# seungju-k1m/Distributed_RL

Measured on AMD Instinct MI355X. Metric: learner frames/sec (whole node), Ape-X DQN Atari CNN, higher is better.
Workload: dtype bf16; 1 GPU; model=ape_x net (ape_x.json), global_batch=512, seq_len=4, parallelism=dp1, actors=0, replay=gpu sum-tree PER, graph=True

## Files before the change

distributed_rl_amd/algos/ape_x.py:

```python

from __future__ import annotations

import os as _os
import time
from collections import deque
from typing import Any, Dict, List, Optional

import numpy as np
import torch

from .. import ops
from ..config import Config
from ..models import BaseAgent
from ..models.base_agent import CNN2D
from ..replay import make_apex_schema, make_per
from .common import LearnerBase

PUBLISH_EVERY = 50
ACTOR_PULL_EVERY = 100


class ApexLearner(LearnerBase):
    ALG = "APE_X"

# ... 408 lines not shown
            t_hid = self._t_pre_hidden_of if pre else self._t_hidden_of
            h_s = hid(f_s)
            with torch.no_grad():
                h_on = hid(f_on)
                h_tg = t_hid(f_tg)
            wa, ba, wv, bv = self._head_params
            wat, bat, wvt, bvt = self._thead_params
            loss, prio, qmean = ops.dueling_q_head_loss(
                h_s, wa, ba, wv, bv, h_on, h_tg, wat, bat, wvt, bvt,
                actions, rewards, dones, weights, self.gamma, self.n_step,
                self.alpha, pre_act=pre,
            )
        elif cuda and getattr(self, "_fast_heads", None) is not None:
            adv_s, val_s = self._fast_heads(s)
            with torch.no_grad():
                adv_on, val_on = self._fast_heads(sp)
                adv_tg, val_tg = self._target_heads(sp)
            loss, prio, qmean = ops.dueling_nstep_dqn_loss(
                adv_s, val_s, adv_on, val_on, adv_tg, val_tg, actions,
                rewards, dones, weights, self.gamma, self.n_step, self.alpha,
            )
        else:
            q_s = self._online_q(s) if cuda else self.net.forward([s])[0]
            with torch.no_grad():
                q_sp_on = (self._online_q(sp) if cuda
                           else self.net.forward([sp])[0])
                q_sp_tg = self.target.forward([sp])[0]
            loss, prio, qmean = ops.nstep_dqn_loss(
                q_s, q_sp_on, q_sp_tg, actions, rewards,
                dones, weights, self.gamma, self.n_step, self.alpha,
                with_value_stat=True,
            )
        if self.mp is not None:
            self.mp.direct_grads(loss, getattr(self, "_direct_list", None))
        else:
            self.optim.zero_grad(set_to_none=False)
            loss.backward()
        return {"loss": loss.detach(), "value": qmean}, prio

    def _optimize_mp(self):
        if (_os.environ.get("DRL_FUSED_OPT_TAIL", "1") == "1"
                and self.mp.fused_step(self.optim)):
            return
        self.mp.upcast_grads()
        self.optim.step()
        self.mp.sync_compute_params()

    def sync_target(self):
        if self.mp is not None:
            self.flat_tparam.copy_(self.mp.flat_cparam)
        else:
            self.target.updateParameter(self.model, 1.0)

    def _inner_step(self) -> Dict[str, torch.Tensor]:
        data, idx, w = self.replay.sample(self.batch_size, self.beta)
        return self.train_step(data, idx, w)

    def _cadence(self):
        self.step_count += 1
        if self.step_count % self.cfg.target_frequency == 0:
            self.sync_target()
            self.publish_weights(include_target=True)
        elif self.step_count % PUBLISH_EVERY == 0:
            self.publish_weights()

    def step(self) -> Dict[str, torch.Tensor]:
        stats = self.maybe_profile_first_step(self._inner_step)
# ... 425 lines not shown
```

distributed_rl_amd/ops/__init__.py:

```python

from __future__ import annotations

import os
from typing import Optional

import torch

from . import torch_ref

_EXT = None
_EXT_TRIED = False


def hip_ext(required: bool = True):
    global _EXT, _EXT_TRIED
    if _EXT is None and not _EXT_TRIED:
        _EXT_TRIED = True
        from . import build as _build

        _EXT = _build.load_prebuilt()
        if _EXT is None and torch.cuda.is_available():
            try:
                _EXT = _build.build()
            except Exception as e:
                if required:
                    raise RuntimeError(
                        "gfx950 HIP extension missing and build failed: %s" % e
                    )
    if _EXT is None and required and not _allow_eager():
        raise RuntimeError(
            "device tensor reached a fused op but the _drl_hip extension is "
            "not built; run `python -m distributed_rl_amd.ops.build` "
            "(or set DRL_ALLOW_EAGER=1 to debug with eager torch)"
        )
    return _EXT
# ... 10 lines not shown
    return ext is not None




def dequant_frames(x_u8: torch.Tensor, dtype: torch.dtype = torch.bfloat16) -> torch.Tensor:
    if _use_hip(x_u8):
        out = torch.empty(x_u8.shape, dtype=dtype, device=x_u8.device)
        hip_ext().dequant(x_u8.contiguous(), out)
        return out
    return torch_ref.dequant_frames(x_u8, dtype)


def dequant_frames_nhwc(x_u8: torch.Tensor) -> torch.Tensor:
    if _use_hip(x_u8):
        out = torch.empty(
            x_u8.shape, dtype=torch.bfloat16, device=x_u8.device,
            memory_format=torch.channels_last,
        )
        hip_ext().dequant_nhwc(x_u8.contiguous(), out)
        return out
    return torch_ref.dequant_frames(x_u8, torch.float32).to(
        memory_format=torch.channels_last
    )




def conv_supported(H, W, C, KH, KW, S, COUT, u8: bool, chw_out: bool = False,
                   njobs: int = 1) -> bool:
    ext = hip_ext(required=False)
    return ext is not None and bool(
        ext.conv_fwd_supported(H, W, C, KH, KW, S, COUT, u8, chw_out, njobs))


def _fused_conv_backward(x, weight, out, gout, stride, has_bias, chw, pq,
                         need_x, need_w, need_b):
    COUT = weight.shape[0]
    if chw:
        P, Q = pq
        N = gout.shape[0]
        masked = torch.empty(N, COUT, P, Q, dtype=torch.bfloat16,
                             device=gout.device,
                             memory_format=torch.channels_last)
        hip_ext().relu_mask_bwd_chw(gout.contiguous(), out, masked,
                                    COUT, P * Q)
        gout = masked
    else:
        if not gout.is_contiguous(memory_format=torch.channels_last):
            gout = gout.contiguous(memory_format=torch.channels_last)
        masked = torch.empty_like(gout)
        hip_ext().relu_mask_bwd(gout, out, masked)
        gout = masked
    COUT, C, KH, KW = weight.shape
    ext = hip_ext()
    use_own_wrw = need_w and bool(
        ext.conv_wrw_supported(x.shape[2], x.shape[3], C, KH, KW, stride,
                               COUT, x.dtype == torch.uint8)
    )
    gw = gb = None
    if use_own_wrw and os.environ.get("DRL_WRW_BF16", "1") == "1":
        gw = torch.empty(COUT, KH, KW, C, dtype=torch.bfloat16,
                         device=x.device).permute(0, 3, 1, 2)
        gb = (torch.empty(COUT, dtype=torch.bfloat16, device=x.device)
              if need_b else None)
        ext.conv_wrw(x, gout, gw,
                     gb if need_b else torch.empty(0, device=x.device),
                     stride)
    elif use_own_wrw:
        K = KH * KW * C
        flat_ws = torch.empty(COUT * (K + 1), dtype=torch.float32,
                              device=x.device)
        ws = flat_ws[: COUT * K].view(COUT, K)
        gb_ws = (flat_ws[COUT * K :] if need_b
                 else torch.empty(0, device=x.device))
        ext.conv_wrw(x, gout, ws, gb_ws, stride)
        gw = ws.view(COUT, KH, KW, C).permute(0, 3, 1, 2).to(torch.bfloat16)
        if need_b:
            gb = gb_ws.to(torch.bfloat16)
    gi = None
    use_own_dgrad = (
        os.environ.get("DRL_OWN_DGRAD", "0") == "1"
        and need_x and x.dtype == torch.bfloat16
        and bool(ext.conv_dgrad_supported(x.shape[2], x.shape[3], C, KH,
                                          KW, stride, COUT))
    )
    if use_own_dgrad:
        gi = torch.empty_like(x)
        w_t = torch.empty(weight.numel(), dtype=torch.bfloat16,
                          device=x.device)
        ext.conv_dgrad(gout, weight, w_t, gi, stride)
    if (need_x and not use_own_dgrad) or (need_w and not use_own_wrw):
        if x.dtype == torch.uint8:
            xf = dequant_frames(x.permute(0, 2, 3, 1), torch.bfloat16)
            xf = xf.permute(0, 3, 1, 2)
        else:
            xf = x
        gi2, gw2, gb2 = torch.ops.aten.convolution_backward(
            gout, xf, weight,
            [COUT] if has_bias else None,
            [stride, stride], [0, 0], [1, 1], False, [0, 0], 1,
# ... 63 lines not shown
                continue
            x, weight, out = saved[k : k + 3]
            k += 3
            if gouts[j] is None:
                continue
            need_x = ctx.needs_input_grad[3 + j]
            need_w = ctx.needs_input_grad[3 + n + j]
            need_b = ctx.has_bias and ctx.needs_input_grad[3 + 2 * n + j]
            gi, gw, gb = _fused_conv_backward(
                x, weight, out, gouts[j], ctx.stride, ctx.has_bias, ctx.chw,
                ctx.pq, need_x, need_w, need_b)
            grads[j], grads[n + j], grads[2 * n + j] = gi, gw, gb
        return (None, None, None, *grads)


def fused_conv_relu_grouped(xs, weights, biases, stride: int,
                            chw_out: bool = False):
    n = len(xs)
    assert len(weights) == n and len(biases) == n
    return _FusedConvGroupedFn.apply(stride, bool(chw_out), n, *xs, *weights,
                                     *biases)


def fused_conv_relu(x, weight, bias, stride: int, chw_out: bool = False):
    return _FusedConvGroupedFn.apply(stride, bool(chw_out), 1, x, weight,
                                     bias)[0]




def conv3x3_supported(H, W, C, COUT) -> bool:
    ext = hip_ext(required=False)
    return ext is not None and bool(ext.conv3x3p1_supported(H, W, C, COUT))


def _gate(name: str, default: bool) -> bool:
    v = os.environ.get(name)
    if v is None or v == "":
        return default
    return v == "1"


_RESCONV_WRW_DEFAULT = True
_RESCONV_DGRAD_DEFAULT = True


class _FusedConv3x3Fn(torch.autograd.Function):

    @staticmethod
    def forward(ctx, x, weight, bias, residual, relu_in, relu_out):
        ext = hip_ext()
        N, _, H, W = x.shape
        COUT = weight.shape[0]
        empty = torch.empty(0, device=x.device, dtype=torch.bfloat16)
        out = torch.empty(
            N, COUT, H, W, dtype=torch.bfloat16, device=x.device,
            memory_format=torch.channels_last,
        )
        ext.conv3x3p1_fwd(x, weight, bias if bias is not None else empty,
                          residual if residual is not None else empty, out,
                          relu_in, relu_out)
        ctx.save_for_backward(x, weight, out if relu_out else None)
        ctx.has_bias = bias is not None
        ctx.relu_in = relu_in
        ctx.relu_out = relu_out
        return out

    @staticmethod
    def backward(ctx, gout):
        x, weight, out = ctx.saved_tensors
        ext = hip_ext()
        COUT = weight.shape[0]
        if not gout.is_contiguous(memory_format=torch.channels_last):
# ... 676 lines not shown
```

distributed_rl_amd/ops/hip/conv_mfma.hip:

```cpp

#include <hip/hip_runtime.h>
#include <atomic>
#include <hip/hip_bf16.h>
#include <torch/extension.h>
#include <ATen/cuda/CUDAContext.h>

namespace {

using bf16x8 = __attribute__((ext_vector_type(8))) __bf16;
using f32x4 = __attribute__((ext_vector_type(4))) float;

constexpr int kPad = 32;

template <int H, int W, int C, int KH, int KW, int S, int COUT, bool U8IN>
struct ConvGeom {
  static constexpr int P = (H - KH) / S + 1;
  static constexpr int Q = (W - KW) / S + 1;
  static constexpr int K = KH * KW * C;
  static constexpr int KCHUNKS = K / 32;
  static_assert(K % 32 == 0, "K must be a multiple of 32");
  static_assert((KW * C) % 32 == 0, "patch row must tile by 32");
  static constexpr int ROWC = KW * C;
  static constexpr int LDS_ROW = K + kPad;
  static constexpr int LDS_ELEMS = COUT * LDS_ROW;
};

template <int H, int W, int C, int KH, int KW, int S, int COUT, bool U8IN,
          int WAVES, int RPW, bool CHW_OUT = false>
__device__ __forceinline__ void conv_fwd_block(
    const void* __restrict__ in_v,
    const __bf16* __restrict__ weight,
    const __bf16* __restrict__ bias,
    __bf16* __restrict__ out,
    int batch, int tile, __bf16* wlds) {
  using G = ConvGeom<H, W, C, KH, KW, S, COUT, U8IN>;
// ... 250 lines not shown
        bf16x8 v;
        if (m < M) {
          v = *reinterpret_cast<const bf16x8*>(gout + (int64_t)m * COUT + c0);
        } else {
#pragma unroll
          for (int j = 0; j < 8; ++j) v[j] = (__bf16)0.0f;
        }
        *reinterpret_cast<bf16x8*>(g_t + (piece / PIECES) * GSTRIDE + c0) = v;
      }
    }
    __syncthreads();
    bf16x8 bfrag = tr_frag<ASTRIDE>(a_t, lane, wave);
#pragma unroll
    for (int cb = 0; cb < CBLK; ++cb) {
      bf16x8 afrag = tr_frag<GSTRIDE>(g_t, lane, cb);
      acc[cb] = __builtin_amdgcn_mfma_f32_16x16x32_bf16(afrag, bfrag, acc[cb],
                                                        0, 0, 0);
    }
    __syncthreads();
  }

  float* plane = gw_part + (int64_t)mb * (COUT * G::K + kPlanePad);
  const int kout = ktile * 64 + wave * 16 + (lane & 15);
#pragma unroll
  for (int cb = 0; cb < CBLK; ++cb)
#pragma unroll
    for (int r = 0; r < 4; ++r) {
      const int cout = cb * 16 + (lane >> 4) * 4 + r;
      plane[(int64_t)cout * G::K + kout] = acc[cb][r];
    }
}

template <typename OutT>
__global__ __launch_bounds__(256) void wrw_reduce_kernel(
    const float* __restrict__ part, int planes, int n_elem,
    OutT* __restrict__ out, const float* __restrict__ b_part, int b_planes,
    int cout, OutT* __restrict__ b_out) {
  __shared__ __attribute__((aligned(16))) float sh4_raw[256 * 4];
  float* sh = sh4_raw;
  const int tid = threadIdx.x;
  const int e_blocks = (n_elem + 63) / 64;
  if ((int)blockIdx.x < e_blocks) {
    const int e4 = blockIdx.x * 64 + (tid & 15) * 4;
    const int g = tid >> 4;
    float4 s = {0.0f, 0.0f, 0.0f, 0.0f};
    const float4 zero = {0.0f, 0.0f, 0.0f, 0.0f};
    for (int p = g; p < planes; p += 64) {
      float4 v[4];
#pragma unroll
      for (int u = 0; u < 4; ++u) {
        const int pu = p + 16 * u;
        v[u] = pu < planes ? *reinterpret_cast<const float4*>(
                                 part + (int64_t)pu * (n_elem + kPlanePad) + e4)
                           : zero;
      }
#pragma unroll
      for (int u = 0; u < 4; ++u) {
        s.x += v[u].x; s.y += v[u].y; s.z += v[u].z; s.w += v[u].w;
      }
    }
    float4* sh4 = reinterpret_cast<float4*>(sh4_raw);
    sh4[tid] = s;
    __syncthreads();
    if (tid < 16) {
      float4 t = sh4[tid];
      for (int k = 1; k < 16; ++k) {
        const float4 v = sh4[k * 16 + tid];
        t.x += v.x; t.y += v.y; t.z += v.z; t.w += v.w;
      }
      if constexpr (std::is_same<OutT, float>::value) {
        *reinterpret_cast<float4*>(out + e4) = t;
      } else {
        v4bf_w o = {(__bf16)t.x, (__bf16)t.y, (__bf16)t.z, (__bf16)t.w};
        *reinterpret_cast<v4bf_w*>(out + e4) = o;
      }
    }
  } else {
    const int G = 256 / cout;
    const int c = tid % cout, g = tid / cout;
    float s = 0.0f;
    for (int p = g; p < b_planes; p += G) s += b_part[p * cout + c];
    sh[tid] = s;
    __syncthreads();
    if (tid < cout) {
      float t = 0.0f;
      for (int k = 0; k < G; ++k) t += sh[k * cout + tid];
      b_out[tid] = (OutT)t;
    }
  }
}

template <int COUT>
__global__ __launch_bounds__(256) void colsum_bf16_kernel(
    const __bf16* __restrict__ x, int64_t M, float* __restrict__ out) {
  typedef __bf16 bf8 __attribute__((ext_vector_type(8)));
  __shared__ float sh[256 * 8];
  const int tid = threadIdx.x;
  const int64_t nchunk = M * COUT / 8;
  int64_t i = (int64_t)blockIdx.x * blockDim.x + tid;
  const int64_t stride = (int64_t)gridDim.x * blockDim.x;
  float acc[8] = {0, 0, 0, 0, 0, 0, 0, 0};
  const bf8* __restrict__ x8 = (const bf8*)x;
  for (; i < nchunk; i += stride) {
    bf8 v = x8[i];
#pragma unroll
    for (int j = 0; j < 8; ++j) acc[j] += (float)v[j];
  }
#pragma unroll
  for (int j = 0; j < 8; ++j) sh[tid * 8 + j] = acc[j];
  __syncthreads();
  if (tid < COUT) {
    float s = 0.0f;
    for (int t = tid >> 3; t < 256; t += COUT / 8) s += sh[t * 8 + (tid & 7)];
    out[(int64_t)blockIdx.x * COUT + tid] = s;
  }
}

}

namespace {
typedef __bf16 v4bf __attribute__((ext_vector_type(4)));
__global__ void tr16_probe_kernel(float* out, int mode) {
  __shared__ __bf16 lds[512];
  int lane = threadIdx.x & 63;
  for (int i = threadIdx.x; i < 512; i += 64) lds[i] = (__bf16)(float)i;
  __syncthreads();
  int off;
  switch (mode) {
    case 0: off = 0; break;
    case 1: off = lane * 4; break;
    case 2: off = (lane >> 4) * 64; break;
    default: off = (lane & 15) * 4; break;
  }
  auto* p = (__attribute__((address_space(3))) v4bf*)(lds + off);
  v4bf v = __builtin_amdgcn_ds_read_tr16_b64_v4bf16(p);
#pragma unroll
  for (int j = 0; j < 4; ++j) out[lane * 4 + j] = (float)v[j];
}
}

namespace {

template <int H, int W, int C, int KH, int KW, int S, int COUT, int WAVES,
          int RPW>
__global__ __launch_bounds__(WAVES * 64) void conv_dgrad_kernel(
    const __bf16* __restrict__ gout,
    const __bf16* __restrict__ w_t,
    __bf16* __restrict__ dx,
    int batch) {
// ... 1205 lines not shown
}

constexpr int kMaxDevices = 64;

int resident_blocks(std::atomic<int>* per_dev, const void* fn, int lds_bytes,
                    const char* who) {
  const int dev = at::cuda::current_device();
  TORCH_CHECK(dev >= 0 && dev < kMaxDevices, who, ": device index");
  std::atomic<int>& slot = per_dev[dev];
  int r = slot.load(std::memory_order_relaxed);
  if (r == 0) {
    int per_cu = 0;
    TORCH_CHECK(hipOccupancyMaxActiveBlocksPerMultiprocessor(
                    &per_cu, fn, 256, lds_bytes) == hipSuccess && per_cu > 0,
                who, ": occupancy query failed");
    r = per_cu * at::cuda::getCurrentDeviceProperties()->multiProcessorCount;
    slot.store(r, std::memory_order_relaxed);
  }
  return r;
}

int wrw_resident_blocks(const Conv3Launch& L) {
  static std::atomic<int> cache[std::size(kConv3Launches)][kMaxDevices] = {};
  return resident_blocks(cache[&L - kConv3Launches], (const void*)L.wrw,
                         L.wrw_lds_bytes, "conv3x3p1_wrw");
}

int wrw_resident_blocks(const StemLaunch& L) {
  static std::atomic<int> cache[std::size(kStemLaunches)][kMaxDevices] = {};
  return resident_blocks(cache[&L - kStemLaunches], (const void*)L.wrw,
                         L.wrw_lds_bytes, "conv3x3c4_wrw");
}

void launch_wrw_fold(const torch::Tensor& part, int mb,
                     const torch::Tensor& gout, int M, int64_t COUT,
                     void (*colsum)(const __bf16*, int64_t, float*),
                     torch::Tensor& gw_ws, torch::Tensor& gb_ws, bool bias) {
  constexpr int kColsumBlocks = 256;
  auto st = cur_stream();
  const int n_elem = (int)gw_ws.numel();
  const bool bf16_out = gw_ws.scalar_type() == kBF16;
  torch::Tensor b_part;
  if (bias) {
    b_part = torch::empty({(int64_t)kColsumBlocks, COUT}, part.options());
    hipLaunchKernelGGL(colsum, dim3(kColsumBlocks), dim3(256), 0, st,
                       (const __bf16*)gout.data_ptr(), (int64_t)M,
                       b_part.data_ptr<float>());
  }
  const int e_blocks = (n_elem + 63) / 64;
  const float* b_part_ptr =
      bias ? (const float*)b_part.data_ptr<float>() : nullptr;
  if (bf16_out)
    hipLaunchKernelGGL(wrw_reduce_kernel<__bf16>,
                       dim3(e_blocks + (bias ? 1 : 0)), dim3(256), 0, st,
                       (const float*)part.data_ptr<float>(), mb, n_elem,
                       (__bf16*)gw_ws.data_ptr(), b_part_ptr, kColsumBlocks,
                       (int)COUT, bias ? (__bf16*)gb_ws.data_ptr() : nullptr);
  else
    hipLaunchKernelGGL(wrw_reduce_kernel<float>,
                       dim3(e_blocks + (bias ? 1 : 0)), dim3(256), 0, st,
                       (const float*)part.data_ptr<float>(), mb, n_elem,
                       gw_ws.data_ptr<float>(), b_part_ptr, kColsumBlocks,
                       (int)COUT, bias ? gb_ws.data_ptr<float>() : nullptr);
}

struct Conv3Labels {
  const char *in, *out, *bias, *residual, *mask;
};

void launch_conv3(const torch::Tensor& in, const __bf16* w,
                  const __bf16* flip_from, const torch::Tensor& bias,
                  const torch::Tensor& residual, const torch::Tensor& mask,
                  const torch::Tensor& out, int64_t COUT, bool relu_in,
                  bool relu_out, const Conv3Labels& lb) {
  const int64_t N = in.size(0), C = in.size(1), H = in.size(2), W = in.size(3);
  check_nhwc(in, kBF16, N, C, H, W, lb.in);
  check_nhwc(out, kBF16, N, COUT, H, W, lb.out);
  TORCH_CHECK(out.data_ptr() != in.data_ptr(), lb.out, " must not alias ",
              lb.in, " (not in-place)");
  TORCH_CHECK((uintptr_t)in.data_ptr() % 16 == 0, lb.in, " is misaligned");
  TORCH_CHECK((uintptr_t)w % 16 == 0, lb.in, "'s weight is misaligned");
// ... 57 lines not shown
                      std::vector<torch::Tensor> biases,
                      std::vector<torch::Tensor> outs, int64_t stride,
                      bool chw_out) {
  const size_t njobs = ins.size();
  TORCH_CHECK(njobs >= 1 && njobs <= kMaxConvJobs, "1..", kMaxConvJobs,
              " conv jobs per launch");
  TORCH_CHECK(weights.size() == njobs && outs.size() == njobs &&
                  (biases.empty() || biases.size() == njobs),
              "conv_fwd_grouped wants one weight, output and bias per job");
  const Geom g = geom_of(ins[0], weights[0], stride);
  const ConvEntry* e = find_geom(kConvs, g);
  TORCH_CHECK(e, "no fused conv kernel for this geometry: ", g.H, "x", g.W,
              "x", g.C, " k", g.KH, "x", g.KW, " s", g.S, " -> ", g.COUT,
              " u8=", g.u8);
  launch_conv_fwd(*e, ins, weights, biases, outs, chw_out);
}

bool conv_fwd_variant(torch::Tensor in, torch::Tensor weight,
                      torch::Tensor bias, torch::Tensor out, int64_t stride,
                      int64_t variant) {
  if (variant < 0 || variant >= (int64_t)std::size(kVariants)) return false;
  const ConvEntry& e = kVariants[variant];
  if (!(e.g == geom_of(in, weight, stride))) return false;
  launch_conv_fwd(e, {in}, {weight}, {bias}, {out}, false);
  return true;
}

bool conv_wrw_supported(int64_t H, int64_t W, int64_t C, int64_t KH, int64_t KW,
                        int64_t S, int64_t COUT, bool u8) {
  const ConvEntry* e = find_conv(H, W, C, KH, KW, S, COUT, u8);
  return e && e->wrw;
}

void conv_wrw(torch::Tensor in, torch::Tensor gout, torch::Tensor gw_ws,
              torch::Tensor gb_ws, int64_t stride) {
  TORCH_CHECK(in.dim() == 4 && gout.dim() == 4 && stride >= 1,
              "conv_wrw wants 4-D in and gout and a positive stride");
  const int64_t N = in.size(0), C = in.size(1), H = in.size(2), W = in.size(3);
  const int64_t COUT = gout.size(1), P = gout.size(2), Q = gout.size(3);
  const bool u8 = in.scalar_type() == torch::kUInt8;
  const ConvEntry* L =
      find_conv(H, W, C, H - (P - 1) * stride, W - (Q - 1) * stride, stride,
                COUT, u8);
  TORCH_CHECK(L && L->wrw, "no wrw kernel for this geometry");
  check_nhwc(in, u8 ? torch::kUInt8 : kBF16, N, C, H, W, "conv_wrw in");
  check_nhwc(gout, kBF16, N, COUT, P, Q, "conv_wrw gout (in's batch)");
  const bool bf16_out = gw_ws.scalar_type() == kBF16;
  check_dev(gw_ws, bf16_out ? kBF16 : torch::kFloat32, "conv_wrw gw_ws");
  TORCH_CHECK(gw_ws.is_contiguous() ||
              (gw_ws.dim() == 4 &&
               gw_ws.is_contiguous(at::MemoryFormat::ChannelsLast)));
  const int n_elem = (int)gw_ws.numel();
  TORCH_CHECK(gw_ws.numel() == COUT * L->g.K(), "gw_ws shape mismatch");
  const bool bias = gb_ws.defined() && gb_ws.numel() > 0;
  if (bias) check_rows(gb_ws, gw_ws.scalar_type(), {COUT}, "conv_wrw gb_ws");
  const int M = checked_rows(N * P * Q, "conv_wrw");
  const int n_chunks = (M + 31) / 32;
  int mb = (n_chunks > 8192 ? 2048 : 512) / L->ktiles;
  if (mb > n_chunks) mb = n_chunks;
  if (mb < 1) mb = 1;
  auto st = cur_stream();
  const auto f32 = gw_ws.options().dtype(torch::kFloat32);
  auto part = torch::empty({(int64_t)mb, (int64_t)n_elem + kPlanePad}, f32);
  hipLaunchKernelGGL(L->wrw, dim3(L->ktiles, mb), dim3(256), L->wrw_lds_bytes,
                     st, (const void*)in.data_ptr(),
                     (const __bf16*)gout.data_ptr(), part.data_ptr<float>(),
                     (int)N, mb);
  launch_wrw_fold(part, mb, gout, M, COUT, L->colsum, gw_ws, gb_ws, bias);
}

bool conv_dgrad_supported(int64_t H, int64_t W, int64_t C, int64_t KH,
                          int64_t KW, int64_t S, int64_t COUT) {
  return find_geom(kDgrad, Geom{H, W, C, KH, KW, S, COUT, false}) != nullptr;
}

void conv_dgrad(torch::Tensor gout, torch::Tensor weight, torch::Tensor w_t,
                torch::Tensor dx, int64_t stride) {
  TORCH_CHECK(dx.dim() == 4 && weight.dim() == 4 && stride >= 1,
              "conv_dgrad wants 4-D dx and weight and a positive stride");
  const int64_t N = dx.size(0), C = dx.size(1), H = dx.size(2), W = dx.size(3);
  const int64_t COUT = weight.size(0), KH = weight.size(2), KW = weight.size(3);
  const DgradEntry* L =
      find_geom(kDgrad, Geom{H, W, C, KH, KW, stride, COUT, false});
  TORCH_CHECK(L, "no dgrad kernel for this geometry");
  check_nhwc(dx, kBF16, N, C, H, W, "conv_dgrad dx");
  check_nhwc(weight, kBF16, COUT, C, KH, KW, "conv_dgrad weight");
  check_nhwc(gout, kBF16, N, COUT, L->g.P(), L->g.Q(), "conv_dgrad gout");
  check_rows(w_t, kBF16, {weight.numel()}, "conv_dgrad w_t");
  const int M = checked_rows(N * H * W, "conv_dgrad");
  if (M == 0) return;
  auto stream = cur_stream();
  const int total = (int)weight.numel();
  hipLaunchKernelGGL(conv_w_transpose_kernel, dim3((total + 255) / 256),
                     dim3(256), 0, stream, (const __bf16*)weight.data_ptr(),
                     (__bf16*)w_t.data_ptr(), (int)(KH * KW), (int)C,
                     (int)COUT);
  const int rows_per_block = L->waves * L->rpw;
  const int blocks = (M + rows_per_block - 1) / rows_per_block;
  hipLaunchKernelGGL(L->fn, dim3(blocks), dim3(L->waves * 64), 0, stream,
                     (const __bf16*)gout.data_ptr(),
                     (const __bf16*)w_t.data_ptr(), (__bf16*)dx.data_ptr(),
                     (int)N);
// ... 268 lines not shown
  const int64_t N = gx.size(0), C = gx.size(1), H = gx.size(2), W = gx.size(3);
  TORCH_CHECK(maxpool3x3s2_supported(H, W, C),
              "no 3x3 s2 max-pool kernel for this geometry: ", H, "x", W, "x",
              C);
  const int64_t P = (H - 1) / 2 + 1, Q = (W - 1) / 2 + 1;
  check_nhwc(gout, kBF16, N, C, P, Q, "maxpool3x3s2_bwd gout");
  check_nhwc(idx, torch::kUInt8, N, C, P, Q, "maxpool3x3s2_bwd idx");
  check_nhwc(gx, kBF16, N, C, H, W, "maxpool3x3s2_bwd gx");
  TORCH_CHECK((uintptr_t)gout.data_ptr() % 16 == 0 &&
                  (uintptr_t)idx.data_ptr() % 16 == 0 &&
                  (uintptr_t)gx.data_ptr() % 16 == 0,
              "maxpool3x3s2_bwd: misaligned tensor");
  const int lanes = checked_rows(N * H * W * (C / 16), "maxpool3x3s2_bwd");
  if (lanes == 0) return;
  const dim3 grid((unsigned)(((int64_t)lanes + 255) / 256));
  hipLaunchKernelGGL(maxpool3x3s2_bwd_kernel, grid, dim3(256), 0, cur_stream(),
                     (const __bf16*)gout.data_ptr(),
                     (const uint8_t*)idx.data_ptr(), (__bf16*)gx.data_ptr(),
                     lanes, (int)H, (int)W, (int)P, (int)Q, (int)(C / 16));
}

void register_conv(pybind11::module_& m) {
  m.def("mfma_probe", &mfma_probe, "16x16x32 bf16 MFMA fragment-map probe");
  m.def("tr16_probe", &tr16_probe);
  m.def("conv_fwd_grouped", &conv_fwd_grouped,
        "fused NHWC bf16 MFMA conv fwd (+dequant on u8 input, bias, ReLU, "
        "optional flatten-fused CHW out) for 1..4 same-geometry jobs in one "
        "launch");
  m.def("conv_fwd_supported", &conv_fwd_supported);
  m.def("conv_fwd_variant", &conv_fwd_variant, "tuning-variant conv fwd");
  m.def("conv_wrw", &conv_wrw,
        "MFMA conv weight-grad; gw/gb are fp32 workspaces or bf16 grads");
  m.def("conv_wrw_supported", &conv_wrw_supported);
  m.def("conv_dgrad", &conv_dgrad,
        "MFMA conv data-grad (masked-tap gather, pre-transposed weights)");
  m.def("conv_dgrad_supported", &conv_dgrad_supported);
  m.def("relu_mask_bwd_chw", &relu_mask_bwd_chw,
        "relu-mask + CHW->NHWC transpose (backward of the fused flatten)");
  m.def("linear_relu", &linear_relu,
        "fused Linear+bias+ReLU fwd (own MFMA GEMM, LDS-staged W)");
  m.def("linear_relu_supported", &linear_relu_supported);
  m.def("conv3x3p1_fwd", &conv3x3p1_fwd,
        "MFMA 3x3 s1 pad-1 NHWC bf16 conv fwd (+relu_in, bias, residual, "
        "relu_out)");
  m.def("conv3x3p1_supported", &conv3x3p1_supported);
  m.def("conv3x3p1_wrw", &conv3x3p1_wrw,
        "MFMA 3x3 s1 pad-1 weight-grad (+relu_in); gw/gb are fp32 workspaces "
        "or bf16 grads");
  m.def("conv3x3p1_wrw_supported", &conv3x3p1_wrw_supported);
  m.def("conv3x3p1_dgrad", &conv3x3p1_dgrad,
        "3x3 s1 pad-1 input-grad: weight flip + the forward kernel at the "
        "mirrored geometry (+relu_in mask in the epilogue)");
  m.def("conv3x3c4_fwd", &conv3x3c4_fwd,
        "MFMA 3x3 s1 pad-1 NHWC bf16 stem conv fwd (84x84, C=4 -> 16; bias)");
  m.def("conv3x3c4_supported", &conv3x3c4_supported);
  m.def("conv3x3c4_wrw", &conv3x3c4_wrw,
        "MFMA stem-conv weight-grad, ordered planes; gw/gb are fp32 "
        "workspaces or bf16 grads");
  m.def("conv3x3c4_wrw_supported", &conv3x3c4_wrw_supported);
  m.def("maxpool3x3s2_fwd", &maxpool3x3s2_fwd,
        "NHWC bf16 max-pool 3x3 s2 pad-1 fwd; uint8 tap plane, or none when "
        "idx is empty");
  m.def("maxpool3x3s2_bwd", &maxpool3x3s2_bwd,
        "max-pool 3x3 s2 pad-1 input-grad: ordered gather over the tap "
        "plane, every gx element written once");
  m.def("maxpool3x3s2_supported", &maxpool3x3s2_supported);
// ... 2 lines not shown
```

distributed_rl_amd/ops/torch_ref.py:

```python

from __future__ import annotations

from typing import Tuple

import torch



def dequant_frames(x_u8: torch.Tensor, dtype: torch.dtype = torch.float32) -> torch.Tensor:
    return x_u8.to(dtype) / 255.0




def conv3x3_res(x, weight, bias=None, relu_in: bool = False,
                relu_out: bool = False, residual=None) -> torch.Tensor:
    y = torch.nn.functional.conv2d(
        torch.nn.functional.relu(x) if relu_in else x, weight, bias, padding=1)
    if residual is not None:
        y = y + residual
    return torch.nn.functional.relu(y) if relu_out else y



# ... 292 lines not shown
def sumtree_bump_seed(seed: int) -> int:
    return ((int(seed) & _U64) * 6364136223846793005
            + 1442695040888963407) & _U64


def sumtree_sample(tree, P: int, n_valid: int, k: int, seed: int):
    import numpy as np

    tree = np.asarray(tree, dtype=np.float32)
    assert tree.size == 2 * P and 1 <= n_valid <= P and k >= 1
    i = np.arange(k, dtype=np.int64)
    total = tree[1]
    u = (i.astype(np.float32) + sumtree_hash01(seed, i)) * (total / np.float32(k))
    node = np.ones(k, dtype=np.int64)
    level = 1
    while level < P:
        left_child = node << 1
        lv = tree[left_child]
        left = u < lv
        u = np.where(left, u, u - lv)
        node = np.where(left, left_child, left_child + 1)
        level <<= 1
    idx = np.minimum(node - P, n_valid - 1)
    prob = tree[P + idx] / total
    return idx, prob




def fold_nstep_reward(rewards: torch.Tensor, gamma: float) -> torch.Tensor:
    n = rewards.shape[-1]
    disc = gamma ** torch.arange(n, dtype=rewards.dtype, device=rewards.device)
    return (rewards * disc).sum(-1)
```

distributed_rl_amd/parallel/precision.py:

```python

from __future__ import annotations

import copy
from typing import Callable, Optional

import torch
import torch.distributed as dist


def _is_cl(p: torch.Tensor) -> bool:
    return p.dim() == 4 and p.is_contiguous(memory_format=torch.channels_last) \
        and not p.is_contiguous()


def _to_flat(p: torch.Tensor) -> torch.Tensor:
    if _is_cl(p):
        return p.permute(0, 2, 3, 1).reshape(-1)
    return p.reshape(-1)


def _view_like(flat_slice: torch.Tensor, p: torch.Tensor) -> torch.Tensor:
    if _is_cl(p):
        N, C, H, W = p.shape
        return flat_slice.view(N, H, W, C).permute(0, 3, 1, 2)
    return flat_slice.view_as(p)


class _Group:

    def __init__(self, dtype, c_params, m_params, device):
        self.dtype = dtype
        self.c_params = c_params
        self.m_params = m_params
        total = sum(p.numel() for p in c_params)
        self.flat_cparam = torch.empty(total, dtype=dtype, device=device)
# ... 66 lines not shown
                    f"params {names} are not adjacent in the flat buffer"
                )
                buf = g.flat_cparam if of == "param" else g.flat_cgrad
                return buf[start:end]
        raise KeyError(f"params {names} not found in one group")

    @property
    def flat_cparam(self):
        assert len(self.groups) == 1
        return self.groups[0].flat_cparam

    @property
    def flat_cgrad(self):
        assert len(self.groups) == 1
        return self.groups[0].flat_cgrad

    @property
    def flat_mgrad(self):
        assert len(self.groups) == 1
        return self.groups[0].flat_mgrad

    @property
    def flat_mparam(self):
        assert len(self.groups) == 1
        return self.groups[0].flat_mparam

    def all_mgrads(self):
        return [g.flat_mgrad for g in self.groups]

    def zero_grads(self):
        for g in self.groups:
            g.flat_cgrad.zero_()

    def direct_grads(self, loss, params_override=None):
        if params_override is not None:
            assert len(self.groups) == 1
            grads = torch.autograd.grad(loss, params_override)
            flats = []
            for p, gr in zip(params_override, grads):
                if gr.dim() == 4 and _is_cl(p) and not _is_cl(gr):
                    gr = gr.contiguous(memory_format=torch.channels_last)
                flats.append(_to_flat(gr))
            torch.cat(flats, out=self.groups[0].flat_cgrad)
            return
        params = [cp for g in self.groups for cp in g.c_params]
        grads = torch.autograd.grad(loss, params)
        i = 0
        for g in self.groups:
            n = len(g.c_params)
            flats = []
            for cp, gr in zip(g.c_params, grads[i : i + n]):
                if gr.dim() == 4 and _is_cl(cp) and not _is_cl(gr):
                    gr = gr.contiguous(memory_format=torch.channels_last)
                flats.append(_to_flat(gr))
            i += n
            torch.cat(flats, out=g.flat_cgrad)

    def allreduce_grads(self):
        if self.world > 1:
            for g in self.groups:
                dist.all_reduce(g.flat_cgrad, group=self.pg)

    def allreduce_grads_async(self):
        if self.world > 1:
            return [dist.all_reduce(g.flat_cgrad, group=self.pg, async_op=True)
                    for g in self.groups]
        return []

    def upcast_grads(self):
        for g in self.groups:
            g.flat_mgrad.copy_(g.flat_cgrad)
            if self.world > 1:
                g.flat_mgrad.mul_(1.0 / self.world)

    def reduce_and_upcast(self):
        self.allreduce_grads()
        self.upcast_grads()

    def sync_compute_params(self):
# ... 22 lines not shown
```

Before: 1.035 million frames/s.

## Defer conv weight-grad fold reductions and batch them into one grouped launch

During backward, each conv weight-grad call now launches only the partial-plane MFMA kernel and the bias colsum, and queues the partials. After autograd finishes, a single grouped reduce kernel folds up to four layers' partials into their bf16 gradients. This removes several small reduce launches per step and gives fewer, larger grids. The cost is that partial buffers stay alive longer, and the gradients are only filled once the context exits. Because of the graph mode, launch savings may be small.

After: 1.090 million frames/s (median of 6 runs). 1.05x the previous value.

```diff
diff --git a/distributed_rl_amd/algos/ape_x.py b/distributed_rl_amd/algos/ape_x.py
--- a/distributed_rl_amd/algos/ape_x.py
+++ b/distributed_rl_amd/algos/ape_x.py
@@ -464,7 +464,8 @@
                 with_value_stat=True,
             )
         if self.mp is not None:
-            self.mp.direct_grads(loss, getattr(self, "_direct_list", None))
+            self.mp.direct_grads(loss, getattr(self, "_direct_list", None),
+                                 defer_wrw=True)
         else:
             self.optim.zero_grad(set_to_none=False)
             loss.backward()
diff --git a/distributed_rl_amd/ops/__init__.py b/distributed_rl_amd/ops/__init__.py
--- a/distributed_rl_amd/ops/__init__.py
+++ b/distributed_rl_amd/ops/__init__.py
@@ -1,6 +1,7 @@
 
 from __future__ import annotations
 
+import contextlib
 import os
 from typing import Optional
 
@@ -77,6 +78,54 @@
     ext = hip_ext(required=False)
     return ext is not None and bool(
         ext.conv_fwd_supported(H, W, C, KH, KW, S, COUT, u8, chw_out, njobs))
+
+
+def _gate(name: str, default: bool) -> bool:
+    v = os.environ.get(name)
+    if v is None or v == "":
+        return default
+    return v == "1"
+
+
+_WRW_DEFER_DEFAULT = True
+
+_MAX_FOLD_JOBS = 4
+
+_pending_wrw_folds = None
+
+
+def _launch_pending_folds(pending) -> None:
+    ext = hip_ext()
+    empty = None
+    for i in range(0, len(pending), _MAX_FOLD_JOBS):
+        jobs = pending[i : i + _MAX_FOLD_JOBS]
+        if empty is None:
+            empty = torch.empty(0, device=jobs[0][3].device)
+        ext.wrw_fold_grouped(
+            [j[0] for j in jobs], [j[1] for j in jobs],
+            [j[2] for j in jobs], [j[3] for j in jobs],
+            [j[4] if j[4] is not None else empty for j in jobs])
+    pending.clear()
+
+
+@contextlib.contextmanager
+def deferred_wrw_folds():
+    global _pending_wrw_folds
+    if (_pending_wrw_folds is not None
+            or not _gate("DRL_WRW_DEFER", _WRW_DEFER_DEFAULT)):
+        yield
+        return
+    pending = []
+    _pending_wrw_folds = pending
+    try:
+        yield
+    except BaseException:
+        pending.clear()
+        raise
+    finally:
+        _pending_wrw_folds = None
+    if pending:
+        _launch_pending_folds(pending)
 
 
 def _fused_conv_backward(x, weight, out, gout, stride, has_bias, chw, pq,
@@ -109,9 +158,14 @@
                          device=x.device).permute(0, 3, 1, 2)
         gb = (torch.empty(COUT, dtype=torch.bfloat16, device=x.device)
               if need_b else None)
-        ext.conv_wrw(x, gout, gw,
-                     gb if need_b else torch.empty(0, device=x.device),
-                     stride)
+        if _pending_wrw_folds is not None:
+            part, mb, b_part = ext.conv_wrw_partials(x, gout, stride,
+                                                     bool(need_b))
+            _pending_wrw_folds.append((part, mb, b_part, gw, gb))
+        else:
+            ext.conv_wrw(x, gout, gw,
+                         gb if need_b else torch.empty(0, device=x.device),
+                         stride)
     elif use_own_wrw:
         K = KH * KW * C
         flat_ws = torch.empty(COUT * (K + 1), dtype=torch.float32,
@@ -241,13 +295,6 @@
 def conv3x3_supported(H, W, C, COUT) -> bool:
     ext = hip_ext(required=False)
     return ext is not None and bool(ext.conv3x3p1_supported(H, W, C, COUT))
-
-
-def _gate(name: str, default: bool) -> bool:
-    v = os.environ.get(name)
-    if v is None or v == "":
-        return default
-    return v == "1"
 
 
 _RESCONV_WRW_DEFAULT = True
diff --git a/distributed_rl_amd/ops/hip/conv_mfma.hip b/distributed_rl_amd/ops/hip/conv_mfma.hip
--- a/distributed_rl_amd/ops/hip/conv_mfma.hip
+++ b/distributed_rl_amd/ops/hip/conv_mfma.hip
@@ -1,6 +1,7 @@
 
 #include <hip/hip_runtime.h>
 #include <atomic>
+#include <tuple>
 #include <hip/hip_bf16.h>
 #include <torch/extension.h>
 #include <ATen/cuda/CUDAContext.h>
@@ -317,16 +318,15 @@
 }
 
 template <typename OutT>
-__global__ __launch_bounds__(256) void wrw_reduce_kernel(
+__device__ __forceinline__ void wrw_reduce_block(
     const float* __restrict__ part, int planes, int n_elem,
     OutT* __restrict__ out, const float* __restrict__ b_part, int b_planes,
-    int cout, OutT* __restrict__ b_out) {
-  __shared__ __attribute__((aligned(16))) float sh4_raw[256 * 4];
+    int cout, OutT* __restrict__ b_out, int block, float* sh4_raw) {
   float* sh = sh4_raw;
   const int tid = threadIdx.x;
   const int e_blocks = (n_elem + 63) / 64;
-  if ((int)blockIdx.x < e_blocks) {
-    const int e4 = blockIdx.x * 64 + (tid & 15) * 4;
+  if (block < e_blocks) {
+    const int e4 = block * 64 + (tid & 15) * 4;
     const int g = tid >> 4;
     float4 s = {0.0f, 0.0f, 0.0f, 0.0f};
     const float4 zero = {0.0f, 0.0f, 0.0f, 0.0f};
@@ -373,6 +373,43 @@
       b_out[tid] = (OutT)t;
     }
   }
+}
+
+template <typename OutT>
+__global__ __launch_bounds__(256) void wrw_reduce_kernel(
+    const float* __restrict__ part, int planes, int n_elem,
+    OutT* __restrict__ out, const float* __restrict__ b_part, int b_planes,
+    int cout, OutT* __restrict__ b_out) {
+  __shared__ __attribute__((aligned(16))) float sh4_raw[256 * 4];
+  wrw_reduce_block<OutT>(part, planes, n_elem, out, b_part, b_planes, cout,
+                         b_out, (int)blockIdx.x, sh4_raw);
+}
+
+constexpr int kMaxFoldJobs = 4;
+template <typename OutT>
+struct WrwFoldJobs {
+  const float* part[kMaxFoldJobs];
+  OutT* out[kMaxFoldJobs];
+  const float* b_part[kMaxFoldJobs];
+  OutT* b_out[kMaxFoldJobs];
+  int planes[kMaxFoldJobs], n_elem[kMaxFoldJobs];
+  int b_planes[kMaxFoldJobs], cout[kMaxFoldJobs];
+  int end_block[kMaxFoldJobs];
+};
+
+template <typename OutT>
+__global__ __launch_bounds__(256) void wrw_reduce_grouped_kernel(
+    const WrwFoldJobs<OutT> jobs, int njobs) {
+  __shared__ __attribute__((aligned(16))) float sh4_raw[256 * 4];
+  const int b = blockIdx.x;
+  int job = 0;
+#pragma unroll
+  for (int j = 0; j < kMaxFoldJobs - 1; ++j)
+    if (j + 1 < njobs && b >= jobs.end_block[j]) job = j + 1;
+  const int first = job == 0 ? 0 : jobs.end_block[job - 1];
+  wrw_reduce_block<OutT>(jobs.part[job], jobs.planes[job], jobs.n_elem[job],
+                         jobs.out[job], jobs.b_part[job], jobs.b_planes[job],
+                         jobs.cout[job], jobs.b_out[job], b - first, sh4_raw);
 }
 
 template <int COUT>
@@ -400,6 +437,8 @@
     out[(int64_t)blockIdx.x * COUT + tid] = s;
   }
 }
+
+constexpr int kColsumBlocks = 256;
 
 }
 
@@ -1671,21 +1710,30 @@
                          L.wrw_lds_bytes, "conv3x3c4_wrw");
 }
 
+void launch_wrw_reduce(const torch::Tensor& part, int mb,
+                       const torch::Tensor& b_part, int64_t COUT,
+                       torch::Tensor& gw_ws, torch::Tensor& gb_ws, bool bias);
+
 void launch_wrw_fold(const torch::Tensor& part, int mb,
                      const torch::Tensor& gout, int M, int64_t COUT,
                      void (*colsum)(const __bf16*, int64_t, float*),
                      torch::Tensor& gw_ws, torch::Tensor& gb_ws, bool bias) {
-  constexpr int kColsumBlocks = 256;
+  torch::Tensor b_part;
+  if (bias) {
+    b_part = torch::empty({(int64_t)kColsumBlocks, COUT}, part.options());
+    hipLaunchKernelGGL(colsum, dim3(kColsumBlocks), dim3(256), 0,
+                       cur_stream(), (const __bf16*)gout.data_ptr(),
+                       (int64_t)M, b_part.data_ptr<float>());
+  }
+  launch_wrw_reduce(part, mb, b_part, COUT, gw_ws, gb_ws, bias);
+}
+
+void launch_wrw_reduce(const torch::Tensor& part, int mb,
+                       const torch::Tensor& b_part, int64_t COUT,
+                       torch::Tensor& gw_ws, torch::Tensor& gb_ws, bool bias) {
   auto st = cur_stream();
   const int n_elem = (int)gw_ws.numel();
   const bool bf16_out = gw_ws.scalar_type() == kBF16;
-  torch::Tensor b_part;
-  if (bias) {
-    b_part = torch::empty({(int64_t)kColsumBlocks, COUT}, part.options());
-    hipLaunchKernelGGL(colsum, dim3(kColsumBlocks), dim3(256), 0, st,
-                       (const __bf16*)gout.data_ptr(), (int64_t)M,
-                       b_part.data_ptr<float>());
-  }
   const int e_blocks = (n_elem + 63) / 64;
   const float* b_part_ptr =
       bias ? (const float*)b_part.data_ptr<float>() : nullptr;
@@ -1809,8 +1857,16 @@
   return e && e->wrw;
 }
 
-void conv_wrw(torch::Tensor in, torch::Tensor gout, torch::Tensor gw_ws,
-              torch::Tensor gb_ws, int64_t stride) {
+namespace {
+
+struct WrwCall {
+  const ConvEntry* L;
+  int64_t N, COUT;
+  int M;
+};
+
+WrwCall check_wrw_inputs(const torch::Tensor& in, const torch::Tensor& gout,
+                         int64_t stride) {
   TORCH_CHECK(in.dim() == 4 && gout.dim() == 4 && stride >= 1,
               "conv_wrw wants 4-D in and gout and a positive stride");
   const int64_t N = in.size(0), C = in.size(1), H = in.size(2), W = in.size(3);
@@ -1822,29 +1878,187 @@
   TORCH_CHECK(L && L->wrw, "no wrw kernel for this geometry");
   check_nhwc(in, u8 ? torch::kUInt8 : kBF16, N, C, H, W, "conv_wrw in");
   check_nhwc(gout, kBF16, N, COUT, P, Q, "conv_wrw gout (in's batch)");
-  const bool bf16_out = gw_ws.scalar_type() == kBF16;
-  check_dev(gw_ws, bf16_out ? kBF16 : torch::kFloat32, "conv_wrw gw_ws");
-  TORCH_CHECK(gw_ws.is_contiguous() ||
-              (gw_ws.dim() == 4 &&
-               gw_ws.is_contiguous(at::MemoryFormat::ChannelsLast)));
-  const int n_elem = (int)gw_ws.numel();
-  TORCH_CHECK(gw_ws.numel() == COUT * L->g.K(), "gw_ws shape mismatch");
-  const bool bias = gb_ws.defined() && gb_ws.numel() > 0;
-  if (bias) check_rows(gb_ws, gw_ws.scalar_type(), {COUT}, "conv_wrw gb_ws");
-  const int M = checked_rows(N * P * Q, "conv_wrw");
+  TORCH_CHECK((uintptr_t)in.data_ptr() % 16 == 0 &&
+                  (uintptr_t)gout.data_ptr() % 16 == 0,
+              "conv_wrw: misaligned tensor");
+  return WrwCall{L, N, COUT, checked_rows(N * P * Q, "conv_wrw")};
+}
+
+struct FoldJob {
+  int planes, n_elem, b_planes, cout;
+  bool bias;
+};
+
+FoldJob check_fold_out(const torch::Tensor& gw, const torch::Tensor& gb,
+                       at::ScalarType dtype) {
+  TORCH_CHECK(gw.defined(), "wrw fold gw is undefined");
+  TORCH_CHECK(dtype == kBF16 || dtype == torch::kFloat32,
+              "wrw fold writes fp32 or bf16");
+  check_dev(gw, dtype, "wrw fold gw");
+  TORCH_CHECK(gw.is_contiguous() ||
+                  (gw.dim() == 4 &&
+                   gw.is_contiguous(at::MemoryFormat::ChannelsLast)),
+              "wrw fold gw must be dense in (cout, kh, kw, c) order");
+  const int64_t n_elem = gw.numel();
+  TORCH_CHECK(n_elem > 0 && n_elem % 64 == 0 && n_elem < ((int64_t)1 << 30),
+              "wrw fold gw must hold a positive multiple of 64 elements");
+  TORCH_CHECK((uintptr_t)gw.data_ptr() % 16 == 0, "wrw fold gw is misaligned");
+  FoldJob j{0, (int)n_elem, 0, 0, gb.defined() && gb.numel() > 0};
+  if (j.bias) {
+    const int64_t cout = gb.numel();
+    TORCH_CHECK(cout <= 256 && 256 % cout == 0,
+                "wrw fold bias: cout must divide 256");
+    check_rows(gb, dtype, {cout}, "wrw fold gb");
+    TORCH_CHECK(gb.device() == gw.device(), "wrw fold: tensors on two devices");
+    j.cout = (int)cout;
+  }
+  return j;
+}
+
+FoldJob check_fold_job(const torch::Tensor& part, int64_t mb,
+                       const torch::Tensor& b_part, const torch::Tensor& gw,
+                       const torch::Tensor& gb, at::ScalarType dtype) {
+  FoldJob j = check_fold_out(gw, gb, dtype);
+  const int64_t n_elem = j.n_elem;
+  TORCH_CHECK(mb >= 1 && mb < ((int64_t)1 << 20), "wrw fold wants >= 1 plane");
+  check_rows(part, torch::kFloat32, {mb, n_elem + kPlanePad},
+             "wrw fold partial planes");
+  TORCH_CHECK((uintptr_t)part.data_ptr() % 16 == 0,
+              "wrw fold partial planes are misaligned");
+  TORCH_CHECK(part.device() == gw.device(), "wrw fold: tensors on two devices");
+  j.planes = (int)mb;
+  const bool has_b_part = b_part.defined() && b_part.numel() > 0;
+  TORCH_CHECK(j.bias == has_b_part,
+              "wrw fold wants b_part and gb together or neither");
+  if (j.bias) {
+    const int64_t cout = j.cout;
+    TORCH_CHECK(b_part.dim() == 2 && b_part.size(0) >= 1 &&
+                    b_part.size(0) < ((int64_t)1 << 20),
+                "wrw fold b_part must be (b_planes, cout)");
+    check_rows(b_part, torch::kFloat32, {b_part.size(0), cout},
+               "wrw fold b_part");
+    TORCH_CHECK(b_part.device() == gw.device(),
+                "wrw fold: tensors on two devices");
+    j.b_planes = (int)b_part.size(0);
+  }
+  return j;
+}
+
+int wrw_mblocks(const ConvEntry& L, int M) {
   const int n_chunks = (M + 31) / 32;
-  int mb = (n_chunks > 8192 ? 2048 : 512) / L->ktiles;
+  int mb = (n_chunks > 8192 ? 2048 : 512) / L.ktiles;
   if (mb > n_chunks) mb = n_chunks;
   if (mb < 1) mb = 1;
+  return mb;
+}
+
+struct WrwPartials {
+  torch::Tensor part, b_part;
+  int mb;
+};
+
+WrwPartials launch_wrw_partials(const WrwCall& c, const torch::Tensor& in,
+                                const torch::Tensor& gout, bool want_bias) {
+  const ConvEntry& L = *c.L;
+  const int mb = wrw_mblocks(L, c.M);
+  const int64_t n_elem = c.COUT * L.g.K();
+  const auto f32 = gout.options().dtype(torch::kFloat32);
+  WrwPartials r;
+  r.mb = mb;
+  r.part = torch::empty({(int64_t)mb, n_elem + kPlanePad}, f32);
   auto st = cur_stream();
-  const auto f32 = gw_ws.options().dtype(torch::kFloat32);
-  auto part = torch::empty({(int64_t)mb, (int64_t)n_elem + kPlanePad}, f32);
-  hipLaunchKernelGGL(L->wrw, dim3(L->ktiles, mb), dim3(256), L->wrw_lds_bytes,
-                     st, (const void*)in.data_ptr(),
-                     (const __bf16*)gout.data_ptr(), part.data_ptr<float>(),
-                     (int)N, mb);
-  launch_wrw_fold(part, mb, gout, M, COUT, L->colsum, gw_ws, gb_ws, bias);
-}
+  hipLaunchKernelGGL(L.wrw, dim3(L.ktiles, mb), dim3(256), L.wrw_lds_bytes, st,
+                     (const void*)in.data_ptr(),
+                     (const __bf16*)gout.data_ptr(), r.part.data_ptr<float>(),
+                     (int)c.N, mb);
+  if (want_bias) {
+    r.b_part = torch::empty({(int64_t)kColsumBlocks, c.COUT}, f32);
+    hipLaunchKernelGGL(L.colsum, dim3(kColsumBlocks), dim3(256), 0, st,
+                       (const __bf16*)gout.data_ptr(), (int64_t)c.M,
+                       r.b_part.data_ptr<float>());
+  }
+  return r;
+}
+
+template <typename OutT>
+void launch_fold_grouped(const std::vector<FoldJob>& jobs,
+                         const std::vector<torch::Tensor>& parts,
+                         const std::vector<torch::Tensor>& b_parts,
+                         const std::vector<torch::Tensor>& gws,
+                         const std::vector<torch::Tensor>& gbs) {
+  WrwFoldJobs<OutT> t{};
+  int blocks = 0;
+  for (size_t j = 0; j < jobs.size(); ++j) {
+    t.part[j] = parts[j].data_ptr<float>();
+    t.out[j] = (OutT*)gws[j].data_ptr();
+    t.b_part[j] = jobs[j].bias ? b_parts[j].data_ptr<float>() : nullptr;
+    t.b_out[j] = jobs[j].bias ? (OutT*)gbs[j].data_ptr() : nullptr;
+    t.planes[j] = jobs[j].planes;
+    t.n_elem[j] = jobs[j].n_elem;
+    t.b_planes[j] = jobs[j].b_planes;
+    t.cout[j] = jobs[j].cout;
+    blocks += jobs[j].n_elem / 64 + (jobs[j].bias ? 1 : 0);
+    t.end_block[j] = blocks;
+  }
+  hipLaunchKernelGGL(wrw_reduce_grouped_kernel<OutT>, dim3(blocks), dim3(256),
+                     0, cur_stream(), t, (int)jobs.size());
+}
+
+}
+
+void conv_wrw(torch::Tensor in, torch::Tensor gout, torch::Tensor gw_ws,
+              torch::Tensor gb_ws, int64_t stride) {
+  const WrwCall c = check_wrw_inputs(in, gout, stride);
+  TORCH_CHECK(gw_ws.defined(), "conv_wrw gw_ws is undefined");
+  const bool bias = check_fold_out(gw_ws, gb_ws, gw_ws.scalar_type()).bias;
+  TORCH_CHECK(gw_ws.numel() == c.COUT * c.L->g.K(), "gw_ws shape mismatch");
+  if (bias)
+    check_rows(gb_ws, gw_ws.scalar_type(), {c.COUT}, "conv_wrw gb_ws");
+  TORCH_CHECK(gw_ws.device() == gout.device(), "conv_wrw: two devices");
+  WrwPartials r = launch_wrw_partials(c, in, gout, bias);
+  const FoldJob job = check_fold_job(r.part, r.mb, r.b_part, gw_ws, gb_ws,
+                                     gw_ws.scalar_type());
+  if (gw_ws.scalar_type() == kBF16)
+    launch_fold_grouped<__bf16>({job}, {r.part}, {r.b_part}, {gw_ws}, {gb_ws});
+  else
+    launch_fold_grouped<float>({job}, {r.part}, {r.b_part}, {gw_ws}, {gb_ws});
+}
+
+std::tuple<torch::Tensor, int64_t, torch::Tensor> conv_wrw_partials(
+    torch::Tensor in, torch::Tensor gout, int64_t stride, bool want_bias) {
+  const WrwCall c = check_wrw_inputs(in, gout, stride);
+  WrwPartials r = launch_wrw_partials(c, in, gout, want_bias);
+  if (!want_bias) r.b_part = torch::empty({0}, r.part.options());
+  return {r.part, (int64_t)r.mb, r.b_part};
+}
+
+void wrw_fold_grouped(std::vector<torch::Tensor> parts,
+                      std::vector<int64_t> mbs,
+                      std::vector<torch::Tensor> b_parts,
+                      std::vector<torch::Tensor> gws,
+                      std::vector<torch::Tensor> gbs) {
+  const size_t n = parts.size();
+  TORCH_CHECK(n >= 1 && n <= (size_t)kMaxFoldJobs, "1..", kMaxFoldJobs,
+              " fold jobs per launch");
+  TORCH_CHECK(mbs.size() == n && b_parts.size() == n && gws.size() == n &&
+                  gbs.size() == n,
+              "wrw_fold_grouped wants one entry per job in every list");
+  TORCH_CHECK(gws[0].defined(), "wrw fold gw is undefined");
+  const at::ScalarType dtype = gws[0].scalar_type();
+  std::vector<FoldJob> jobs;
+  for (size_t j = 0; j < n; ++j) {
+    jobs.push_back(
+        check_fold_job(parts[j], mbs[j], b_parts[j], gws[j], gbs[j], dtype));
+    TORCH_CHECK(gws[j].device() == gws[0].device(),
+                "wrw fold: jobs on two devices");
+  }
+  if (dtype == kBF16)
+    launch_fold_grouped<__bf16>(jobs, parts, b_parts, gws, gbs);
+  else
+    launch_fold_grouped<float>(jobs, parts, b_parts, gws, gbs);
+}
+
+int64_t wrw_plane_pad() { return kPlanePad; }
 
 bool conv_dgrad_supported(int64_t H, int64_t W, int64_t C, int64_t KH,
                           int64_t KW, int64_t S, int64_t COUT) {
@@ -2179,6 +2393,11 @@
   m.def("conv_wrw", &conv_wrw,
         "MFMA conv weight-grad; gw/gb are fp32 workspaces or bf16 grads");
   m.def("conv_wrw_supported", &conv_wrw_supported);
+  m.def("conv_wrw_partials", &conv_wrw_partials,
+        "wrw launch only -> (part, mb, b_part) for wrw_fold_grouped");
+  m.def("wrw_fold_grouped", &wrw_fold_grouped,
+        "ordered fold of up to 4 weight gradients in one launch");
+  m.def("wrw_plane_pad", &wrw_plane_pad);
   m.def("conv_dgrad", &conv_dgrad,
         "MFMA conv data-grad (masked-tap gather, pre-transposed weights)");
   m.def("conv_dgrad_supported", &conv_dgrad_supported);
diff --git a/distributed_rl_amd/ops/torch_ref.py b/distributed_rl_amd/ops/torch_ref.py
--- a/distributed_rl_amd/ops/torch_ref.py
+++ b/distributed_rl_amd/ops/torch_ref.py
@@ -348,3 +348,35 @@
     n = rewards.shape[-1]
     disc = gamma ** torch.arange(n, dtype=rewards.dtype, device=rewards.device)
     return (rewards * disc).sum(-1)
+
+
+
+
+def wrw_fold_ordered(part: torch.Tensor, n_elem: int, b_part=None,
+                     out_dtype: torch.dtype = torch.float32):
+    p = part.detach().to("cpu", torch.float32)[:, :n_elem]
+    planes = p.shape[0]
+    sums = []
+    for g in range(16):
+        s = torch.zeros(n_elem, dtype=torch.float32)
+        for k in range(g, planes, 16):
+            s = s + p[k]
+        sums.append(s)
+    t = sums[0]
+    for g in range(1, 16):
+        t = t + sums[g]
+    gw = t.to(out_dtype)
+    gb = None
+    if b_part is not None:
+        b = b_part.detach().to("cpu", torch.float32)
+        b_planes, cout = b.shape
+        assert 256 % cout == 0
+        G = 256 // cout
+        tb = torch.zeros(cout, dtype=torch.float32)
+        for g in range(G):
+            s = torch.zeros(cout, dtype=torch.float32)
+            for k in range(g, b_planes, G):
+                s = s + b[k]
+            tb = tb + s
+        gb = tb.to(out_dtype)
+    return gw, gb
diff --git a/distributed_rl_amd/parallel/precision.py b/distributed_rl_amd/parallel/precision.py
--- a/distributed_rl_amd/parallel/precision.py
+++ b/distributed_rl_amd/parallel/precision.py
@@ -1,6 +1,7 @@
 
 from __future__ import annotations
 
+import contextlib
 import copy
 from typing import Callable, Optional
 
@@ -133,10 +134,16 @@
         for g in self.groups:
             g.flat_cgrad.zero_()
 
-    def direct_grads(self, loss, params_override=None):
+    def direct_grads(self, loss, params_override=None, defer_wrw=False):
+        if defer_wrw:
+            from ..ops import deferred_wrw_folds
+            backward_ctx = deferred_wrw_folds
+        else:
+            backward_ctx = contextlib.nullcontext
         if params_override is not None:
             assert len(self.groups) == 1
-            grads = torch.autograd.grad(loss, params_override)
+            with backward_ctx():
+                grads = torch.autograd.grad(loss, params_override)
             flats = []
             for p, gr in zip(params_override, grads):
                 if gr.dim() == 4 and _is_cl(p) and not _is_cl(gr):
@@ -145,7 +152,8 @@
             torch.cat(flats, out=self.groups[0].flat_cgrad)
             return
         params = [cp for g in self.groups for cp in g.c_params]
-        grads = torch.autograd.grad(loss, params)
+        with backward_ctx():
+            grads = torch.autograd.grad(loss, params)
         i = 0
         for g in self.groups:
             n = len(g.c_params)
```
